# davidbau/rewriting

Measured on AMD Instinct MI355X. Metric: images/sec StyleGANv2-1024 fwd, higher is better.
Workload: dtype f32 (conv operands split into exact f16 pairs from 32x32 up, f32 accumulate); 1 GPU; stylegan2-1024 generator forward (FFHQ-1024 architecture); batch_per_gpu=64, mconv=seq, weights=synthetic seed 0, parallelism=seeds partitioned per rank, no collective, matrix_mode=split, direct_sums=auto

## Files before the change

include/rewriting_hip.h:

```cpp
#ifndef REWRITING_HIP_H
#define REWRITING_HIP_H

#include <stdint.h>

#ifdef __cplusplus
extern "C" {
#endif

typedef void* rw_stream_t;

#define RW_ERR_BAD_ARGUMENT 10001
#define RW_ERR_UNSUPPORTED  10002

int rw_abi_version(void);
const char* rw_error_string(int code);


int rw_fused_bias_act_f32(const float* x, const float* b, const float* ref, float* y,
                          int64_t n, int64_t step_b, int64_t size_b,
                          int act, int grad, float alpha, float scale, rw_stream_t stream);
int rw_fused_bias_act_f16(const uint16_t* x, const uint16_t* b, const uint16_t* ref, uint16_t* y,
                          int64_t n, int64_t step_b, int64_t size_b,
                          int act, int grad, float alpha, float scale, rw_stream_t stream);
int rw_fused_bias_act_f64(const double* x, const double* b, const double* ref, double* y,
// ... 9 lines not shown

int rw_upfirdn2d_f32(const float* x, const float* k, float* y,
                     int major, int in_h, int in_w, int minor, int kh, int kw,
                     int up_x, int up_y, int down_x, int down_y,
                     int pad_x0, int pad_x1, int pad_y0, int pad_y1, rw_stream_t stream);
int rw_upfirdn2d_f16(const uint16_t* x, const uint16_t* k, uint16_t* y,
                     int major, int in_h, int in_w, int minor, int kh, int kw,
                     int up_x, int up_y, int down_x, int down_y,
                     int pad_x0, int pad_x1, int pad_y0, int pad_y1, rw_stream_t stream);
int rw_upfirdn2d_f64(const double* x, const double* k, double* y,
                     int major, int in_h, int in_w, int minor, int kh, int kw,
                     int up_x, int up_y, int down_x, int down_y,
                     int pad_x0, int pad_x1, int pad_y0, int pad_y1, rw_stream_t stream);


int rw_pixel_norm_f32(const float* x, float* y, int batch, int dim, float eps, rw_stream_t stream);

int rw_equal_linear_f32(const float* x, const float* w, const float* bias, float* y,
                        int batch, int in_dim, int out_dim, int64_t x_stride,
                        float w_scale, float b_scale, int act, float alpha, float act_scale,
                        rw_stream_t stream);

int rw_adjust_latent_f32(const float* w, const float* avg, float* out, int batch, int n_latent,
                         int dim, float psi, rw_stream_t stream);

int rw_style_mul_f32(const float* x, const float* style, float* y, int batch, int channels,
                     int64_t hw, rw_stream_t stream);

int rw_weight_sqsum_f32(const float* w, float* wsq, int out_ch, int in_ch, int taps, float w_scale,
                        rw_stream_t stream);

int rw_demod_f32(const float* wsq, const float* style, float* demod, int batch, int out_ch,
                 int in_ch, float eps, rw_stream_t stream);

long long rw_packed_conv_weight_elems(int out_ch, int in_ch, int mode);
int rw_pack_conv_weight_f32(const float* w, float* wp, int out_ch, int in_ch, int mode,
                            rw_stream_t stream);

typedef struct rw_conv_epilogue {
  const float* style;
  const float* demod;
  const float* noise;
  const float* noise_w;
  const float* bias;
  int act;
} rw_conv_epilogue;

int rw_conv3x3_f32(const float* x, const float* wp, float* y, int batch, int in_ch, int out_ch,
                   int h, int w, float w_scale, const rw_conv_epilogue* ep, int impl,
                   rw_stream_t stream);

typedef struct rw_rgb_epilogue {
  const float* weight;
  const float* style;
  const float* bias;
  const float* skip;
  float* out;
  float scale;
} rw_rgb_epilogue;
int rw_conv3x3_to_rgb_f32(const float* x, const float* wp, float* y, int batch, int in_ch, int out_ch,
                          int h, int w, float w_scale, const rw_conv_epilogue* ep,
                          const rw_rgb_epilogue* rgb, rw_stream_t stream);

long long rw_packed_conv_weight_bf16x3_bytes(int out_ch, int in_ch);
int rw_pack_conv_weight_bf16x3(const float* w, void* wb, int out_ch, int in_ch, rw_stream_t stream);
int rw_conv3x3_bf16x6_f32(const float* x, const void* wb, float* y, int batch, int in_ch, int out_ch,
// ... 341 lines not shown
```

rewriting_amd/_lib.py:

```python
import ctypes
import os
from ctypes import (POINTER, Structure, c_char_p, c_double, c_float, c_int, c_int32, c_int64, c_uint,
                    c_void_p)

_HERE = os.path.dirname(os.path.abspath(__file__))
LIB_PATH = os.environ.get('RW_HIP_LIB') or os.path.join(_HERE, 'librewriting_hip.so')

ABI_VERSION = 11


class ConvEpilogue(Structure):
    _fields_ = [('style', c_void_p), ('demod', c_void_p), ('noise', c_void_p),
                ('noise_w', c_void_p), ('bias', c_void_p), ('act', c_int)]


class RgbEpilogue(Structure):
    _fields_ = [('weight', c_void_p), ('style', c_void_p), ('bias', c_void_p), ('skip', c_void_p),
                ('out', c_void_p), ('scale', c_float)]


LPIPS_MAX_TAPS = 8


class LpipsMaps(Structure):
    _fields_ = [('d', c_void_p * LPIPS_MAX_TAPS), ('h', c_int * LPIPS_MAX_TAPS), ('w', c_int * LPIPS_MAX_TAPS), ('n', c_int)]


LpipsGradMaps = LpipsMaps


class SolveProblem(Structure):
    _fields_ = [
        ('out_ch', c_int), ('in_ch', c_int), ('h', c_int), ('w', c_int), ('rank', c_int),
        ('key', c_void_p), ('style', c_void_p), ('val', c_void_p), ('bias', c_void_p),
        ('noise', c_void_p), ('noise_w', c_void_p), ('context', c_void_p), ('ortho', c_void_p),
        ('weight', c_void_p), ('exp_avg', c_void_p), ('exp_avg_sq', c_void_p),
        ('step_size', c_void_p), ('bc2_sqrt', c_void_p), ('step_counter', c_void_p),
        ('losses', c_void_p),
        ('conv', c_void_p), ('wsq', c_void_p), ('gd', c_void_p), ('c2', c_void_p),
        ('grad', c_void_p),
        ('ksplit', c_int), ('beta1', c_float), ('beta2', c_float), ('eps', c_float),
        ('w_scale', c_float), ('low_rank_gradient', c_int),
        ('one_minus_beta1', c_float), ('one_minus_beta2', c_float),
        ('upsample', c_int), ('blur_k', c_void_p), ('linear_insert', c_int), ('lambda_', c_void_p),
    ]


SIGNATURES = {
    'rw_abi_version': (c_int, []),
    'rw_error_string': (c_char_p, [c_int]),
    'rw_fused_bias_act_f32': (c_int, [c_void_p, c_void_p, c_void_p, c_void_p, c_int64, c_int64,
                                      c_int64, c_int, c_int, c_float, c_float, c_void_p]),
    'rw_fused_bias_act_f16': (c_int, [c_void_p, c_void_p, c_void_p, c_void_p, c_int64, c_int64,
                                      c_int64, c_int, c_int, c_float, c_float, c_void_p]),
    'rw_fused_bias_act_f64': (c_int, [c_void_p, c_void_p, c_void_p, c_void_p, c_int64, c_int64,
                                      c_int64, c_int, c_int, c_double, c_double, c_void_p]),
    'rw_bias_grad_f32': (c_int, [c_void_p, c_void_p, c_int64, c_int64, c_int64, c_void_p]),
    'rw_bias_grad_f16': (c_int, [c_void_p, c_void_p, c_int64, c_int64, c_int64, c_void_p]),
    'rw_bias_grad_f64': (c_int, [c_void_p, c_void_p, c_int64, c_int64, c_int64, c_void_p]),
    'rw_upfirdn2d_f32': (c_int, [c_void_p, c_void_p, c_void_p] + [c_int] * 14 + [c_void_p]),
    'rw_upfirdn2d_f16': (c_int, [c_void_p, c_void_p, c_void_p] + [c_int] * 14 + [c_void_p]),
    'rw_upfirdn2d_f64': (c_int, [c_void_p, c_void_p, c_void_p] + [c_int] * 14 + [c_void_p]),
    'rw_pixel_norm_f32': (c_int, [c_void_p, c_void_p, c_int, c_int, c_float, c_void_p]),
    'rw_equal_linear_f32': (c_int, [c_void_p, c_void_p, c_void_p, c_void_p, c_int, c_int, c_int,
                                    c_int64, c_float, c_float, c_int, c_float, c_float, c_void_p]),
    'rw_adjust_latent_f32': (c_int, [c_void_p, c_void_p, c_void_p, c_int, c_int, c_int, c_float,
                                     c_void_p]),
    'rw_style_mul_f32': (c_int, [c_void_p, c_void_p, c_void_p, c_int, c_int, c_int64, c_void_p]),
    'rw_weight_sqsum_f32': (c_int, [c_void_p, c_void_p, c_int, c_int, c_int, c_float, c_void_p]),
    'rw_demod_f32': (c_int, [c_void_p, c_void_p, c_void_p, c_int, c_int, c_int, c_float, c_void_p]),
    'rw_packed_conv_weight_elems': (ctypes.c_longlong, [c_int, c_int, c_int]),
    'rw_pack_conv_weight_f32': (c_int, [c_void_p, c_void_p, c_int, c_int, c_int, c_void_p]),
    'rw_conv3x3_f32': (c_int, [c_void_p, c_void_p, c_void_p, c_int, c_int, c_int, c_int, c_int,
                               c_float, POINTER(ConvEpilogue), c_int, c_void_p]),
    'rw_packed_conv_weight_bf16x3_bytes': (ctypes.c_longlong, [c_int, c_int]),
    'rw_pack_conv_weight_bf16x3': (c_int, [c_void_p, c_void_p, c_int, c_int, c_void_p]),
    'rw_conv3x3_bf16x6_f32': (c_int, [c_void_p, c_void_p, c_void_p, c_int, c_int, c_int, c_int, c_int,
                                      c_float, POINTER(ConvEpilogue), c_void_p]),
    'rw_conv3x3_to_rgb_f32': (c_int, [c_void_p, c_void_p, c_void_p, c_int, c_int, c_int, c_int, c_int,
                                      c_float, POINTER(ConvEpilogue), POINTER(RgbEpilogue), c_void_p]),
    'rw_conv_transpose3x3s2_f32': (c_int, [c_void_p, c_void_p, c_void_p, c_int, c_int, c_int, c_int,
                                           c_int, c_float, POINTER(ConvEpilogue), c_int, c_void_p]),
    'rw_noise_add_f32': (c_int, [c_void_p, c_void_p, c_void_p, c_void_p, c_int, c_int, c_int64,
                                 c_void_p]),
    'rw_blur_noise_act_f32': (c_int, [c_void_p, c_void_p, c_void_p, c_void_p, c_void_p, c_void_p,
                                      c_int, c_int, c_int, c_int, c_void_p]),
    'rw_to_rgb_f32': (c_int, [c_void_p, c_void_p, c_void_p, c_void_p, c_void_p, c_void_p, c_int,
                              c_int, c_int64, c_float, c_void_p]),
    'rw_second_moment_workspace_bytes': (c_int64, [c_int, c_int64]),
    'rw_second_moment_f32': (c_int, [c_void_p, c_void_p, c_int64, c_int, c_int64, c_int, c_void_p,
                                     c_void_p]),
    'rw_channel_sums_f32': (c_int, [c_void_p, c_void_p, c_int64, c_int, c_int64, c_int, c_int,
                                    c_void_p]),
    'rw_channel_moments_f32': (c_int, [c_void_p, c_void_p, c_int64, c_int, c_int64, c_int, c_int,
                                       c_void_p]),
    'rw_key_response_f32': (c_int, [c_void_p, c_void_p, c_void_p, c_void_p, c_int64, c_int, c_int64, c_int,
                                    c_void_p]),
    'rw_render_bytes_f32': (c_int, [c_void_p, c_void_p, c_void_p, c_int64, c_int, c_int, c_int, c_int, c_int, c_float,
                                    c_int, c_uint, c_int32, c_float, c_void_p]),
    'rw_png_segment_bytes': (c_int64, []),
    'rw_png_segment_capacity': (c_int64, []),
    'rw_png_table_words': (c_int64, []),
    'rw_png_filter_u8': (c_int, [c_void_p] * 6 + [c_int64, c_int, c_int, c_void_p]),
# ... 183 lines not shown
```

rewriting_amd/csrc/rw_ops.hip:

```cpp
#include "rw_common.h"
#include <stdlib.h>
#include <stdint.h>

extern "C" int rw_abi_version(void) { return 11; }

extern "C" const char* rw_error_string(int code) {
  if (code == 0) return "success";
  if (code == RW_ERR_BAD_ARGUMENT) return "rewriting_hip: bad argument";
  if (code == RW_ERR_UNSUPPORTED) return "rewriting_hip: unsupported configuration";
  return hipGetErrorString((hipError_t)code);
}

template <typename T> struct RwAcc { typedef T type; };
template <> struct RwAcc<_Float16> { typedef float type; };

template <typename A>
__device__ __forceinline__ A rw_bias_act_one(A x, A ref, int code, A alpha, A scale) {
  A y;
  switch (code) {
    default:
    case 10: y = x; break;
    case 11: y = x; break;
    case 12: y = A(0); break;
    case 30: y = (x > A(0)) ? x : x * alpha; break;
// ... 393 lines not shown
    wr[j] = (j < per && i < in_dim) ? w[(int64_t)o * in_dim + i] * w_scale : 0.f;
  }
  const float bv = bias ? bias[o] * b_scale : 0.f;
  for (int b0 = blockIdx.y * RW_LINEAR_ROWS; b0 < batch; b0 += gridDim.y * RW_LINEAR_ROWS) {
    float acc[RW_LINEAR_ROWS];
#pragma unroll
    for (int r = 0; r < RW_LINEAR_ROWS; ++r) {
      acc[r] = 0.f;
      const int b = b0 + r;
      if (b < batch) {
        const float* xr = x + (int64_t)b * x_stride;
#pragma unroll
        for (int j = 0; j < RW_LINEAR_MAX_PER_LANE; ++j) {
          const int i = lane + j * 64;
          if (j < per && i < in_dim) acc[r] += xr[i] * wr[j];
        }
      }
    }
#pragma unroll
    for (int off = 32; off > 0; off >>= 1)
#pragma unroll
      for (int r = 0; r < RW_LINEAR_ROWS; ++r) acc[r] += __shfl_xor(acc[r], off, 64);
    if (lane < RW_LINEAR_ROWS && b0 + lane < batch) {
      float v = acc[0];
#pragma unroll
      for (int r = 1; r < RW_LINEAR_ROWS; ++r) v = (lane == r) ? acc[r] : v;
      v += bv;
      if (act) v = ((v > 0.f) ? v : v * alpha) * act_scale;
      y[(int64_t)(b0 + lane) * out_dim + o] = v;
    }
  }
}

__global__ void __launch_bounds__(64) equal_linear_mfma_kernel(
    const float* __restrict__ x, const float* __restrict__ w, const float* __restrict__ bias,
    float* __restrict__ y, int batch, int in_dim, int out_dim, int64_t x_stride, float w_scale,
    float b_scale, int act, float alpha, float act_scale) {
  const int lane = threadIdx.x, mn = lane & 15, q = lane >> 4;
  const int o0 = blockIdx.x * 16, b0 = blockIdx.y * 16;
  const int brow = min(b0 + mn, batch - 1);
  const float* xp = x + (int64_t)brow * x_stride + 4 * q;
  const float* wp = w + (int64_t)(o0 + mn) * in_dim + 4 * q;
  rw_f32x4 acc = {0.f, 0.f, 0.f, 0.f};
  const int blocks = in_dim >> 4;
  constexpr int DEPTH = 8;
  for (int c0 = 0; c0 < blocks; c0 += DEPTH) {
    rw_f32x4 a[DEPTH], b[DEPTH];
#pragma unroll
    for (int d = 0; d < DEPTH; ++d) {
      const int c = min(c0 + d, blocks - 1);
      a[d] = *reinterpret_cast<const rw_f32x4*>(xp + 16 * c);
      b[d] = *reinterpret_cast<const rw_f32x4*>(wp + 16 * c);
    }
#pragma unroll
    for (int d = 0; d < DEPTH; ++d) {
      if (c0 + d < blocks) {
        const rw_f32x4 bs = b[d] * w_scale;
#pragma unroll
        for (int j = 0; j < 4; ++j) acc = __builtin_amdgcn_mfma_f32_16x16x4f32(a[d][j], bs[j], acc, 0, 0, 0);
      }
    }
  }
  const int o = o0 + mn;
  const float bv = bias ? bias[o] * b_scale : 0.f;
#pragma unroll
  for (int j = 0; j < 4; ++j) {
    const int b = b0 + 4 * q + j;
    if (b < batch) {
      float v = acc[j] + bv;
      if (act) v = ((v > 0.f) ? v : v * alpha) * act_scale;
      y[(int64_t)b * out_dim + o] = v;
    }
  }
}

extern "C" int rw_equal_linear_f32(const float* x, const float* w, const float* bias, float* y,
                                   int batch, int in_dim, int out_dim, int64_t x_stride,
                                   float w_scale, float b_scale, int act, float alpha,
                                   float act_scale, rw_stream_t stream) {
  RW_CHECK_ARG(x && w && y && batch > 0 && in_dim > 0 && out_dim > 0 && x_stride >= in_dim);
  const char* impl = getenv("RW_LINEAR_IMPL");
  const bool butterfly = impl && atoi(impl) == 1;
  if (!butterfly && in_dim % 16 == 0 && out_dim % 16 == 0 && x_stride % 4 == 0 && ((uintptr_t)x & 15) == 0 &&
      ((uintptr_t)w & 15) == 0) {
    hipLaunchKernelGGL(equal_linear_mfma_kernel, dim3(out_dim / 16, (batch + 15) / 16), dim3(64), 0, rw_s(stream), x,
                       w, bias, y, batch, in_dim, out_dim, x_stride, w_scale, b_scale, act, alpha, act_scale);
    return RW_LAUNCH_RESULT();
  }
  if (in_dim > 64 * RW_LINEAR_MAX_PER_LANE) return RW_ERR_UNSUPPORTED;
  int gy = (batch + RW_LINEAR_ROWS - 1) / RW_LINEAR_ROWS;
  if (gy > 64) gy = 64;
  hipLaunchKernelGGL(equal_linear_kernel, dim3((out_dim + 3) / 4, gy), dim3(256), 0, rw_s(stream), x, w,
                     bias, y, batch, in_dim, out_dim, x_stride, w_scale, b_scale, act, alpha,
                     act_scale);
  return RW_LAUNCH_RESULT();
}

__global__ void __launch_bounds__(256) adjust_latent_kernel(const float* __restrict__ w,
                                                            const float* __restrict__ avg,
                                                            float* __restrict__ out, int batch,
                                                            int n_latent, int dim, float psi) {
  const int64_t total = (int64_t)batch * n_latent * dim;
  for (int64_t idx = (int64_t)blockIdx.x * blockDim.x + threadIdx.x; idx < total;
       idx += (int64_t)gridDim.x * blockDim.x) {
    const int d = (int)(idx % dim);
    const int b = (int)(idx / ((int64_t)n_latent * dim));
    float v = w[(int64_t)b * dim + d];
    if (avg) { const float a = avg[d]; v = a + psi * (v - a); }
    out[idx] = v;
  }
}

extern "C" int rw_adjust_latent_f32(const float* w, const float* avg, float* out, int batch,
                                    int n_latent, int dim, float psi, rw_stream_t stream) {
  RW_CHECK_ARG(w && out && batch > 0 && n_latent > 0 && dim > 0);
  const int64_t total = (int64_t)batch * n_latent * dim;
  hipLaunchKernelGGL(adjust_latent_kernel, dim3(rw_stream_grid(total, 256)), dim3(256), 0,
// ... 61 lines not shown
       i += (int64_t)gridDim.x * blockDim.x) {
    float acc = 0.f;
    for (int t = 0; t < taps; ++t) { const float v = w_scale * w[i * taps + t]; acc += v * v; }
    wsq[i] = acc;
  }
}

extern "C" int rw_weight_sqsum_f32(const float* w, float* wsq, int out_ch, int in_ch, int taps,
                                   float w_scale, rw_stream_t stream) {
  RW_CHECK_ARG(w && wsq && out_ch > 0 && in_ch > 0 && taps > 0);
  const int64_t pairs = (int64_t)out_ch * in_ch;
  hipLaunchKernelGGL(weight_sqsum_kernel, dim3(rw_stream_grid(pairs, 256)), dim3(256), 0,
                     rw_s(stream), w, wsq, pairs, taps, w_scale);
  return RW_LAUNCH_RESULT();
}

__global__ void __launch_bounds__(256) demod_kernel(const float* __restrict__ wsq,
                                                    const float* __restrict__ style,
                                                    float* __restrict__ demod, int batch, int out_ch,
                                                    int in_ch, float eps) {
  const int64_t idx = (int64_t)blockIdx.x * 4 + (threadIdx.x >> 6);
  const int lane = threadIdx.x & 63;
  if (idx >= (int64_t)batch * out_ch) return;
  const int b = (int)(idx / out_ch), o = (int)(idx % out_ch);
  float acc = 0.f;
  for (int i = lane; i < in_ch; i += 64) {
    const float s = style[(int64_t)b * in_ch + i];
    acc += (s * s) * wsq[(int64_t)o * in_ch + i];
  }
  acc = rw_wave_sum(acc);
  if (lane == 0) demod[idx] = rsqrtf(acc + eps);
}

__global__ void __launch_bounds__(64) demod_mfma_kernel(const float* __restrict__ wsq, const float* __restrict__ style,
                                                        float* __restrict__ demod, int batch, int out_ch, int in_ch,
                                                        float eps) {
  const int lane = threadIdx.x, mn = lane & 15, q = lane >> 4;
  const int o0 = blockIdx.x * 16, b0 = blockIdx.y * 16;
  const int brow = min(b0 + mn, batch - 1);
  const float* sp = style + (int64_t)brow * in_ch + 4 * q;
  const float* wp = wsq + (int64_t)(o0 + mn) * in_ch + 4 * q;
  rw_f32x4 acc = {0.f, 0.f, 0.f, 0.f};
  const int blocks = in_ch >> 4;
  constexpr int DEPTH = 8;
  for (int c0 = 0; c0 < blocks; c0 += DEPTH) {
    rw_f32x4 a[DEPTH], b[DEPTH];
#pragma unroll
    for (int d = 0; d < DEPTH; ++d) {
      const int c = min(c0 + d, blocks - 1);
      a[d] = *reinterpret_cast<const rw_f32x4*>(sp + 16 * c);
      b[d] = *reinterpret_cast<const rw_f32x4*>(wp + 16 * c);
    }
#pragma unroll
    for (int d = 0; d < DEPTH; ++d) {
      if (c0 + d < blocks) {
#pragma unroll
        for (int j = 0; j < 4; ++j) acc = __builtin_amdgcn_mfma_f32_16x16x4f32(a[d][j] * a[d][j], b[d][j], acc, 0, 0, 0);
      }
    }
  }
#pragma unroll
  for (int j = 0; j < 4; ++j) {
    const int b = b0 + 4 * q + j;
    if (b < batch) demod[(int64_t)b * out_ch + o0 + mn] = rsqrtf(acc[j] + eps);
  }
}

extern "C" int rw_demod_f32(const float* wsq, const float* style, float* demod, int batch,
                            int out_ch, int in_ch, float eps, rw_stream_t stream) {
  RW_CHECK_ARG(wsq && style && demod && batch > 0 && out_ch > 0 && in_ch > 0);
  const char* impl = getenv("RW_LINEAR_IMPL");
  if (!(impl && atoi(impl) == 1) && in_ch % 16 == 0 && out_ch % 16 == 0 && ((uintptr_t)wsq & 15) == 0 &&
      ((uintptr_t)style & 15) == 0) {
    hipLaunchKernelGGL(demod_mfma_kernel, dim3(out_ch / 16, (batch + 15) / 16), dim3(64), 0, rw_s(stream), wsq, style,
                       demod, batch, out_ch, in_ch, eps);
    return RW_LAUNCH_RESULT();
  }
  const int64_t waves = (int64_t)batch * out_ch;
  hipLaunchKernelGGL(demod_kernel, dim3((unsigned)rw_cdiv(waves, 4)), dim3(256), 0, rw_s(stream),
                     wsq, style, demod, batch, out_ch, in_ch, eps);
  return RW_LAUNCH_RESULT();
}

__constant__ int rw_up_tap_order[9] = {0, 2, 6, 8, 1, 7, 3, 5, 4};

static inline bool rw_frag_ok(int out_ch, int in_ch) { return out_ch % 32 == 0 && in_ch % 16 == 0; }
static inline int rw_frag_ic(int out_ch, int mode) { return (mode == 1 || out_ch % 64 == 0) ? 16 : 8; }

extern "C" long long rw_packed_conv_weight_elems(int out_ch, int in_ch, int mode) {
  if (out_ch <= 0 || in_ch <= 0 || (mode != 0 && mode != 1)) return -1;
  const long long io = (long long)in_ch * out_ch;
  if (!rw_frag_ok(out_ch, in_ch)) return 9 * io;
  return 18 * io;
}

__global__ void __launch_bounds__(256) pack_conv_weight_kernel(const float* __restrict__ w,
                                                               float* __restrict__ wp, int out_ch,
                                                               int in_ch, int mode) {
  const int64_t total = (int64_t)9 * in_ch * out_ch;
  for (int64_t idx = (int64_t)blockIdx.x * blockDim.x + threadIdx.x; idx < total;
       idx += (int64_t)gridDim.x * blockDim.x) {
    const int o = (int)(idx % out_ch);
    const int i = (int)((idx / out_ch) % in_ch);
    const int slab = (int)(idx / ((int64_t)out_ch * in_ch));
    const int tap = mode == 0 ? slab : rw_up_tap_order[slab];
    wp[idx] = w[((int64_t)o * in_ch + i) * 9 + tap];
// ... 402 lines not shown
    for (int i = 0; i < in_ch; ++i) {
      const float v = xb[(int64_t)i * hw + q];
      a[0] += wm[i] * v; a[1] += wm[in_ch + i] * v; a[2] += wm[2 * in_ch + i] * v;
    }
#pragma unroll
    for (int c = 0; c < 3; ++c) {
      const int64_t off = ((int64_t)b * 3 + c) * hw + q;
      float o = a[c] + (bias ? bias[c] : 0.f);
      if (skip) o += skip[off];
      y[off] = o;
    }
  }
}

extern "C" int rw_to_rgb_f32(const float* x, const float* w, const float* style, const float* bias,
                             const float* skip, float* y, int batch, int in_ch, int64_t hw,
                             float w_scale, rw_stream_t stream) {
  RW_CHECK_ARG(x && w && style && y && batch > 0 && in_ch > 0 && hw > 0);
  if (hw % 4) {
    int gs = (int)rw_cdiv(hw, 256);
    if (gs > 2048) gs = 2048;
    hipLaunchKernelGGL(to_rgb_scalar_kernel, dim3(gs, batch), dim3(256), 3 * in_ch * sizeof(float), rw_s(stream), x, w,
                       style, bias, skip, y, in_ch, hw, w_scale);
    return RW_LAUNCH_RESULT();
  }
  int gx = (int)rw_cdiv(hw / 4, 256);
  const int cap = (256 * 8 + batch - 1) / batch;
  if (gx > cap) gx = cap;
  if (gx < 1) gx = 1;
  hipLaunchKernelGGL(to_rgb_kernel, dim3(gx, batch), dim3(256), 3 * in_ch * sizeof(float),
                     rw_s(stream), x, w, style, bias, skip, y, in_ch, hw, w_scale);
  return RW_LAUNCH_RESULT();
}
```

rewriting_amd/hip.py:

```python
import ctypes
from collections import namedtuple as _namedtuple

import torch

from . import _lib
from ._lib import ConvEpilogue, RgbEpilogue, SolveProblem, check

SQRT2 = 2 ** 0.5


def _stream():
    return ctypes.c_void_p(torch.cuda.current_stream().cuda_stream)


def _dev(t, name='tensor', dtype=torch.float32):
    if not isinstance(t, torch.Tensor):
        raise TypeError('%s must be a torch.Tensor' % name)
    if not t.is_cuda:
        raise RuntimeError('rewriting_amd: %s is on %s; the HIP kernels need a GPU tensor '
                           '(there is no CPU fallback)' % (name, t.device))
    if t.dtype != dtype:
        if dtype == torch.float32:
            raise RuntimeError('rewriting_amd: %s is %s; the C ABI is fp32 only (RW_ERR_UNSUPPORTED, include/rewriting_hip.h: '
                               'the reference\'s pybind modules also dispatch half and double, this library does not) -- '
# ... 200 lines not shown
    return y


def pixel_norm(x, eps=1e-8):
    return _pixel_norm_as(torch.float32, x, eps)


def equal_linear(x, weight, bias, w_scale, b_scale, act=False, alpha=0.2, act_scale=SQRT2):
    return _equal_linear_as(torch.float32, x, weight, bias, w_scale, b_scale, act, alpha, act_scale)


def adjust_latent(w, avg, n_latent, psi):
    return _adjust_latent_as(torch.float32, w, avg, n_latent, psi)


def style_mul(x, style):
    return _style_mul_as(torch.float32, x, style)


def weight_sqsum(weight, w_scale):
    return _weight_sqsum_as(torch.float32, weight, w_scale)


def demod(wsq, style, eps=1e-8):
    return _demod_as(torch.float32, wsq, style, eps)


def noise_add(x, noise, noise_w):
    return _noise_add_as(torch.float32, x, noise, noise_w)


def to_rgb(x, weight, style, bias, skip, w_scale):
    return _to_rgb_as(torch.float32, x, weight, style, bias, skip, w_scale)


def blur_noise_act(x, k4, noise, noise_w, bias, post_scale=None, y_amax=None):
    x = _dev(x, 'fmap')
    k4 = _dev(k4, 'blur kernel')
    noise = _opt(noise, 'noise')
    noise_w = _opt(noise_w, 'noise weight')
    bias = _opt(bias, 'bias')
    b, c, ih, iw = x.shape
    y = torch.empty(b, c, ih - 1, iw - 1, device=x.device, dtype=x.dtype)
    post_scale = _post_scale(post_scale, b, c, 'channels')
    y_amax = _amax_out(y_amax, y.numel())
    check(lib().rw_blur_noise_act_amax_f32(_p(x), _p(k4), _p(noise), _p(noise_w), _p(bias), _p(post_scale), _p(y),
                                           b, c, ih - 1, iw - 1, _p(y_amax), _stream()))
    return y


HalfSkip = _namedtuple('HalfSkip', 'image fir')


def _half_skip(skip, b, h, w):
    image, fir = _dev(skip.image, 'rgb skip (half size)'), _dev(skip.fir, 'upsampling kernel')
    if tuple(image.shape) != (b, 3, h // 2, w // 2) or h % 2 or w % 2 or tuple(fir.shape) != (4, 4):
        raise ValueError('half-size rgb skip / kernel shapes')
    return HalfSkip(image, fir)


def rgb_combine(partials, bias, skip):
    partials = _dev(partials, 'rgb partial sums')
    bias = _opt(bias, 'rgb bias')
    n, b, c, h, w = partials.shape
    y = torch.empty(b, 3, h, w, device=partials.device, dtype=partials.dtype)
    if isinstance(skip, HalfSkip):
# ... 1342 lines not shown
```

rewriting_amd/utils/stylegan2/models.py:

```python
import contextlib
import math
import re
import threading
import warnings
from collections import OrderedDict, namedtuple

import numpy as np
import torch
from torch import nn

from . import grad, op, routing
from .routing import switches
from ... import hip


_weight_epoch = [0]


def bump_weight_epoch():
    _weight_epoch[0] += 1


class _DerivedWeights:

# ... 1038 lines not shown
        k = list(self._modules).index('up_rgb%d' % (int(math.log2(from_res)) - 2))
        d = z
        for m in mods[:k]:
            d = m(d)
        total = d.latent.shape[0]
        out = None
        with _scope(final=final):
            for s in range(0, total, mb):
                e = min(s + mb, total)
                part = DataBag({key: (v[s:e] if torch.is_tensor(v) and v.dim() > 0 and v.shape[0] == total else v)
                                for key, v in d.items()})
                part['batch_rows'] = (s, total)
                for m in mods[k:]:
                    part = m(part)
                if out is None:
                    out = part.new_empty((total,) + tuple(part.shape[1:]))
                out[s:e] = part
                del part
        return out

    def _prefetch_modulations(self, d, aux):
        pre = {}
        todo = []
        for name, mod in self._modules.items():
            if not isinstance(mod, nn.Sequential) or isinstance(mod, StyledConvSeq):
                continue
            kids = list(mod.children())
            if len(kids) != 2 or not isinstance(kids[0], PickLatent):
                continue
            if isinstance(kids[1], StyledConvSeq) and kids[1]._fusable() and isinstance(kids[1].mconv, ModulatedConv2dSeq):
                todo.append((kids[0].index, kids[1]))
            elif isinstance(kids[1], ToRGBF):
                todo.append((kids[0].index, kids[1]))
        if len(todo) < 3:
            return {}
        main = torch.cuda.current_stream()
        aux.wait_stream(main)
        with torch.cuda.stream(aux):
            for index, mod in todo[2:]:
                lat = d.latent[:, index]
                if isinstance(mod, ToRGBF):
                    pre[id(mod)] = mod.conv.modulation(lat)
                else:
                    style = mod.mconv.modulation(DataBag(style=lat)).style
                    pre[id(mod)] = (style, mod.mconv.dconv.demod_factors(style))
        return dict(pre=pre, pre_join=aux)

    def _topology(self):
        near, final, prev = {}, None, None
        last = ('layer%d' % (self.num_layers + 1), 'to_rgb%d' % (self.log_size - 1))
        steps = list(self._modules.items())
        for (name, step), (nname, nstep) in zip(steps, steps[1:] + [(None, None)]):
            sconv = getattr(step, 'sconv', None)
            conv = sconv or getattr(step, 'conv', None)
            if not isinstance(conv, StyledConvSeq):
                continue
            if prev is not None:
                near[id(prev)] = near[id(prev)]._replace(reader=conv)
            prev = conv
            kids = list(nstep.children()) if nstep is not None else []
            picks = [m for m in kids if isinstance(m, PickLatent)]
            index = picks[0].index if len(picks) == 1 else None
            leads = index is not None and kids[0] is picks[0]
            nconv, rgb = getattr(nstep, 'sconv', None), getattr(nstep, 'rgb', None)
            successor = torgb = None
            if (conv is sconv and leads and isinstance(nconv, StyledConvSeq)
                    and getattr(conv.mconv, 'upsample', False) and not getattr(nconv.mconv, 'upsample', False)):
                successor = (nconv, index)
            if isinstance(rgb, ToRGBF):
                if leads and len(kids) == 2 and kids[1] is rgb:
                    torgb = (rgb, index)
                if conv is sconv and index is not None and (name, nname) == last:
                    final = (conv, rgb, index)
            near[id(conv)] = _Neighbours(None, successor, torgb)
        return near, final

    def bag_from_z(self, z):
        return InputLatent()(z)

# ... 48 lines not shown
```

rewriting_amd/utils/stylegan2/routing.py:

```python
import os
from collections import namedtuple

from ... import hip

_CONV_IMPLS = {'auto': 0, 'mfma': 0, 'direct': 1, 'generic': 2, 'halo': 3, 'nosplitk': 5}
ONE_PASS_UP_MAX_IN = 64
FUSED_UP_MAX_IN = 512

Switches = namedtuple('Switches', [
    'fuse',
    'conv_impl',
    'conv_precision',
    'conv_algo',
    'up_algo',
    'mm',
    'mm_hooked_split',
    'mm_parts',
    'mm_direct16',
    'micro_batch',
    'up_fused',
    'up_fused2',
    'up_fused2_hooked',
    'up_fused2_max_in',
    'up_fused2_join',
    'direct16_small',
    'direct16_hooked',
    'dconv_ws_fwd',
    'dconv_v',
    'rgb_partial',
    'rgb_f4',
    'rgb_stream',
    'strip_stream',
    'side_priority',
    'prescale',
    'mm_no_handover',
    'prefetch_styles',
    'fuse_final_rgb',
    'rgb_inline_up',
])


def switches():
    env = os.environ.get
    direct16 = env('RW_MM_DIRECT16', 'auto')
    parts = env('RW_MM_PARTS')
    k, _, res = env('RW_MICRO_BATCH', '0').partition(':')
    return Switches(
        fuse=env('RW_FUSE', '1') != '0',
        conv_impl=_CONV_IMPLS[env('RW_CONV_IMPL', 'auto')],
        conv_precision=env('RW_CONV_PRECISION', 'f32'),
        conv_algo=env('RW_CONV_ALGO'),
        up_algo=env('RW_UP_ALGO', 'winograd'),
        mm=env('RW_MM'),
        mm_hooked_split=env('RW_MM_HOOKED', 'split') != 'f32',
        mm_parts=None if parts is None else tuple(parts.split(',')),
        mm_direct16={'auto': ('conv', 'up'), '1': ('conv', 'up', 'rgb')}.get(direct16) or tuple(direct16.split(',')),
        micro_batch=(int(k or 0), int(res or 256)),
        up_fused=env('RW_UP_FUSED', '1') != '0',
        up_fused2=env('RW_UP_FUSED2', '1') == '1',
        up_fused2_hooked=env('RW_UP_FUSED2_HOOKED', '1') == '1',
        up_fused2_max_in=int(env('RW_UP_FUSED2_MAX_IN', FUSED_UP_MAX_IN)),
        up_fused2_join=env('RW_UP_FUSED2_JOIN') == '1',
        direct16_small=env('RW_DIRECT16_SMALL', '1') != '0',
        direct16_hooked=env('RW_DIRECT16_HOOKED', '1') == '1',
        dconv_ws_fwd=env('RW_DCONV_WS_FWD', '1') != '0',
        dconv_v=env('RW_DCONV_V') == '1',
        rgb_partial=env('RW_RGB_PARTIAL', '1') != '0',
        rgb_f4=env('RW_RGB_F4', '1') != '0',
        rgb_stream=env('RW_RGB_STREAM', '1') != '0',
        strip_stream=env('RW_STRIP_STREAM', '1') != '0',
        side_priority=int(env('RW_SIDE_PRIORITY', '0')),
        prescale=env('RW_PRESCALE', '1') != '0',
        mm_no_handover=env('RW_MM_NO_HANDOVER') == '1',
        prefetch_styles=env('RW_PREFETCH_STYLES', '1') != '0',
        fuse_final_rgb=env('RW_FUSE_FINAL_RGB', '1') != '0',
        rgb_inline_up=env('RW_RGB_INLINE_UP', '1') != '0',
    )


Context = namedtuple('Context', 'image_path on_device capturing rgb_stream aux_stream weight_changes')

STRIDE1_KERNELS = ('direct16', 'wino4_split', 'wino4', 'wino', 'bf16x6', 'gemm')
WHOLE_LAYER_KERNELS = ('fused', 'one_pass_direct16', 'one_pass_wino4')
UP_KERNELS = WHOLE_LAYER_KERNELS + ('f22_strips', 'halo_strips', 'plain')

Stride1Route = namedtuple('Stride1Route', 'kernel specialised rgb_partials reads_bound reports_bound prescaled')

UpRoute = namedtuple('UpRoute', 'kernel split side_strips reads_bound runs_layer')

FinalRgbRoute = namedtuple('FinalRgbRoute', 'kernel reads_bound')


def _stride1(kernel, *flags):
    if kernel not in STRIDE1_KERNELS:
        raise ValueError(kernel)
    return Stride1Route(kernel, *flags)


def _up(kernel, *flags):
    if kernel not in UP_KERNELS:
        raise ValueError(kernel)
    return UpRoute(kernel, *flags, kernel in WHOLE_LAYER_KERNELS)


def _final_rgb(kernel, reads_bound):
    if kernel not in STRIDE1_KERNELS:
        raise ValueError(kernel)
# ... 96 lines not shown
```

Measured before the change: 1656 images/sec.

## Batch all style modulation linears and demod factors into grouped kernel launches

Adds grouped kernels that compute every layer's style linear, and every demodulation factor, in a single launch each. A prefix table of tiles tells each block which problem it belongs to. The prefetch path is switched on by default, and it replaces the earlier side-stream prefetch of per-layer modulations. The goal is to cut the many small kernel launches and the Python overhead in the modulation stage. In exchange, the parameter struct passed to the kernel is large, and the per-block problem lookup adds a little work.

```diff
diff --git a/include/rewriting_hip.h b/include/rewriting_hip.h
--- a/include/rewriting_hip.h
+++ b/include/rewriting_hip.h
@@ -65,6 +65,39 @@
 
 int rw_demod_f32(const float* wsq, const float* style, float* demod, int batch, int out_ch,
                  int in_ch, float eps, rw_stream_t stream);
+
+#define RW_GROUP_MAX 32
+typedef struct RwLinearGroup {
+  const float* x[RW_GROUP_MAX];
+  const float* w[RW_GROUP_MAX];
+  const float* bias[RW_GROUP_MAX];
+  float* y[RW_GROUP_MAX];
+  int64_t x_stride[RW_GROUP_MAX];
+  int in_dim[RW_GROUP_MAX];
+  int out_dim[RW_GROUP_MAX];
+  float w_scale[RW_GROUP_MAX];
+  float b_scale[RW_GROUP_MAX];
+  int act[RW_GROUP_MAX];
+  int tile0[RW_GROUP_MAX + 1];
+  int n;
+  int batch;
+  float alpha;
+  float act_scale;
+} RwLinearGroup;
+int rw_equal_linear_group_f32(const RwLinearGroup* g, rw_stream_t stream);
+
+typedef struct RwDemodGroup {
+  const float* wsq[RW_GROUP_MAX];
+  const float* style[RW_GROUP_MAX];
+  float* demod[RW_GROUP_MAX];
+  int out_ch[RW_GROUP_MAX];
+  int in_ch[RW_GROUP_MAX];
+  int tile0[RW_GROUP_MAX + 1];
+  int n;
+  int batch;
+  float eps;
+} RwDemodGroup;
+int rw_demod_group_f32(const RwDemodGroup* g, rw_stream_t stream);
 
 long long rw_packed_conv_weight_elems(int out_ch, int in_ch, int mode);
 int rw_pack_conv_weight_f32(const float* w, float* wp, int out_ch, int in_ch, int mode,
diff --git a/rewriting_amd/_lib.py b/rewriting_amd/_lib.py
--- a/rewriting_amd/_lib.py
+++ b/rewriting_amd/_lib.py
@@ -17,6 +17,24 @@
 class RgbEpilogue(Structure):
     _fields_ = [('weight', c_void_p), ('style', c_void_p), ('bias', c_void_p), ('skip', c_void_p),
                 ('out', c_void_p), ('scale', c_float)]
+
+
+ERR_UNSUPPORTED = 10002
+GROUP_MAX = 32
+
+
+class LinearGroup(Structure):
+    _fields_ = [('x', c_void_p * GROUP_MAX), ('w', c_void_p * GROUP_MAX), ('bias', c_void_p * GROUP_MAX),
+                ('y', c_void_p * GROUP_MAX), ('x_stride', c_int64 * GROUP_MAX), ('in_dim', c_int * GROUP_MAX),
+                ('out_dim', c_int * GROUP_MAX), ('w_scale', c_float * GROUP_MAX), ('b_scale', c_float * GROUP_MAX),
+                ('act', c_int * GROUP_MAX), ('tile0', c_int * (GROUP_MAX + 1)), ('n', c_int), ('batch', c_int),
+                ('alpha', c_float), ('act_scale', c_float)]
+
+
+class DemodGroup(Structure):
+    _fields_ = [('wsq', c_void_p * GROUP_MAX), ('style', c_void_p * GROUP_MAX), ('demod', c_void_p * GROUP_MAX),
+                ('out_ch', c_int * GROUP_MAX), ('in_ch', c_int * GROUP_MAX), ('tile0', c_int * (GROUP_MAX + 1)),
+                ('n', c_int), ('batch', c_int), ('eps', c_float)]
 
 
 LPIPS_MAX_TAPS = 8
@@ -69,6 +87,8 @@
     'rw_style_mul_f32': (c_int, [c_void_p, c_void_p, c_void_p, c_int, c_int, c_int64, c_void_p]),
     'rw_weight_sqsum_f32': (c_int, [c_void_p, c_void_p, c_int, c_int, c_int, c_float, c_void_p]),
     'rw_demod_f32': (c_int, [c_void_p, c_void_p, c_void_p, c_int, c_int, c_int, c_float, c_void_p]),
+    'rw_equal_linear_group_f32': (c_int, [POINTER(LinearGroup), c_void_p]),
+    'rw_demod_group_f32': (c_int, [POINTER(DemodGroup), c_void_p]),
     'rw_packed_conv_weight_elems': (ctypes.c_longlong, [c_int, c_int, c_int]),
     'rw_pack_conv_weight_f32': (c_int, [c_void_p, c_void_p, c_int, c_int, c_int, c_void_p]),
     'rw_conv3x3_f32': (c_int, [c_void_p, c_void_p, c_void_p, c_int, c_int, c_int, c_int, c_int,
diff --git a/rewriting_amd/csrc/rw_ops.hip b/rewriting_amd/csrc/rw_ops.hip
--- a/rewriting_amd/csrc/rw_ops.hip
+++ b/rewriting_amd/csrc/rw_ops.hip
@@ -449,12 +449,10 @@
   }
 }
 
-__global__ void __launch_bounds__(64) equal_linear_mfma_kernel(
-    const float* __restrict__ x, const float* __restrict__ w, const float* __restrict__ bias,
-    float* __restrict__ y, int batch, int in_dim, int out_dim, int64_t x_stride, float w_scale,
-    float b_scale, int act, float alpha, float act_scale) {
+__device__ __forceinline__ void equal_linear_mfma_tile(const float* x, const float* w, const float* bias, float* y,
+                                                       int batch, int in_dim, int out_dim, int64_t x_stride, float w_scale,
+                                                       float b_scale, int act, float alpha, float act_scale, int o0, int b0) {
   const int lane = threadIdx.x, mn = lane & 15, q = lane >> 4;
-  const int o0 = blockIdx.x * 16, b0 = blockIdx.y * 16;
   const int brow = min(b0 + mn, batch - 1);
   const float* xp = x + (int64_t)brow * x_stride + 4 * q;
   const float* wp = w + (int64_t)(o0 + mn) * in_dim + 4 * q;
@@ -491,15 +489,30 @@
   }
 }
 
+__global__ void __launch_bounds__(64) equal_linear_mfma_kernel(
+    const float* __restrict__ x, const float* __restrict__ w, const float* __restrict__ bias,
+    float* __restrict__ y, int batch, int in_dim, int out_dim, int64_t x_stride, float w_scale,
+    float b_scale, int act, float alpha, float act_scale) {
+  equal_linear_mfma_tile(x, w, bias, y, batch, in_dim, out_dim, x_stride, w_scale, b_scale, act, alpha, act_scale,
+                         blockIdx.x * 16, blockIdx.y * 16);
+}
+
+static inline bool rw_linear_mfma_ok(const float* x, const float* w, int in_dim, int out_dim, int64_t x_stride) {
+  return in_dim % 16 == 0 && out_dim % 16 == 0 && x_stride % 4 == 0 && ((uintptr_t)x & 15) == 0 &&
+         ((uintptr_t)w & 15) == 0;
+}
+
+static inline bool rw_linear_butterfly_forced() {
+  const char* impl = getenv("RW_LINEAR_IMPL");
+  return impl && atoi(impl) == 1;
+}
+
 extern "C" int rw_equal_linear_f32(const float* x, const float* w, const float* bias, float* y,
                                    int batch, int in_dim, int out_dim, int64_t x_stride,
                                    float w_scale, float b_scale, int act, float alpha,
                                    float act_scale, rw_stream_t stream) {
   RW_CHECK_ARG(x && w && y && batch > 0 && in_dim > 0 && out_dim > 0 && x_stride >= in_dim);
-  const char* impl = getenv("RW_LINEAR_IMPL");
-  const bool butterfly = impl && atoi(impl) == 1;
-  if (!butterfly && in_dim % 16 == 0 && out_dim % 16 == 0 && x_stride % 4 == 0 && ((uintptr_t)x & 15) == 0 &&
-      ((uintptr_t)w & 15) == 0) {
+  if (!rw_linear_butterfly_forced() && rw_linear_mfma_ok(x, w, in_dim, out_dim, x_stride)) {
     hipLaunchKernelGGL(equal_linear_mfma_kernel, dim3(out_dim / 16, (batch + 15) / 16), dim3(64), 0, rw_s(stream), x,
                        w, bias, y, batch, in_dim, out_dim, x_stride, w_scale, b_scale, act, alpha, act_scale);
     return RW_LAUNCH_RESULT();
@@ -627,11 +640,9 @@
   if (lane == 0) demod[idx] = rsqrtf(acc + eps);
 }
 
-__global__ void __launch_bounds__(64) demod_mfma_kernel(const float* __restrict__ wsq, const float* __restrict__ style,
-                                                        float* __restrict__ demod, int batch, int out_ch, int in_ch,
-                                                        float eps) {
+__device__ __forceinline__ void demod_mfma_tile(const float* wsq, const float* style, float* demod, int batch, int out_ch,
+                                                int in_ch, float eps, int o0, int b0) {
   const int lane = threadIdx.x, mn = lane & 15, q = lane >> 4;
-  const int o0 = blockIdx.x * 16, b0 = blockIdx.y * 16;
   const int brow = min(b0 + mn, batch - 1);
   const float* sp = style + (int64_t)brow * in_ch + 4 * q;
   const float* wp = wsq + (int64_t)(o0 + mn) * in_ch + 4 * q;
@@ -661,12 +672,20 @@
   }
 }
 
+__global__ void __launch_bounds__(64) demod_mfma_kernel(const float* __restrict__ wsq, const float* __restrict__ style,
+                                                        float* __restrict__ demod, int batch, int out_ch, int in_ch,
+                                                        float eps) {
+  demod_mfma_tile(wsq, style, demod, batch, out_ch, in_ch, eps, blockIdx.x * 16, blockIdx.y * 16);
+}
+
+static inline bool rw_demod_mfma_ok(const float* wsq, const float* style, int out_ch, int in_ch) {
+  return in_ch % 16 == 0 && out_ch % 16 == 0 && ((uintptr_t)wsq & 15) == 0 && ((uintptr_t)style & 15) == 0;
+}
+
 extern "C" int rw_demod_f32(const float* wsq, const float* style, float* demod, int batch,
                             int out_ch, int in_ch, float eps, rw_stream_t stream) {
   RW_CHECK_ARG(wsq && style && demod && batch > 0 && out_ch > 0 && in_ch > 0);
-  const char* impl = getenv("RW_LINEAR_IMPL");
-  if (!(impl && atoi(impl) == 1) && in_ch % 16 == 0 && out_ch % 16 == 0 && ((uintptr_t)wsq & 15) == 0 &&
-      ((uintptr_t)style & 15) == 0) {
+  if (!rw_linear_butterfly_forced() && rw_demod_mfma_ok(wsq, style, out_ch, in_ch)) {
     hipLaunchKernelGGL(demod_mfma_kernel, dim3(out_ch / 16, (batch + 15) / 16), dim3(64), 0, rw_s(stream), wsq, style,
                        demod, batch, out_ch, in_ch, eps);
     return RW_LAUNCH_RESULT();
@@ -1135,3 +1154,60 @@
                      rw_s(stream), x, w, style, bias, skip, y, in_ch, hw, w_scale);
   return RW_LAUNCH_RESULT();
 }
+
+
+__device__ __forceinline__ int rw_group_problem(const int* tile0, int n, int t) {
+  int p = 0;
+  while (p + 1 < n && t >= tile0[p + 1]) ++p;
+  return p;
+}
+
+__device__ __forceinline__ int rw_group_out(const RwLinearGroup& g, int p) { return g.out_dim[p]; }
+__device__ __forceinline__ int rw_group_out(const RwDemodGroup& g, int p) { return g.out_ch[p]; }
+
+__device__ __forceinline__ void rw_group_tile(const RwLinearGroup& g, int p, int o0, int b0) {
+  equal_linear_mfma_tile(g.x[p], g.w[p], g.bias[p], g.y[p], g.batch, g.in_dim[p], g.out_dim[p], g.x_stride[p],
+                         g.w_scale[p], g.b_scale[p], g.act[p], g.alpha, g.act_scale, o0, b0);
+}
+
+__device__ __forceinline__ void rw_group_tile(const RwDemodGroup& g, int p, int o0, int b0) {
+  demod_mfma_tile(g.wsq[p], g.style[p], g.demod[p], g.batch, g.out_ch[p], g.in_ch[p], g.eps, o0, b0);
+}
+
+template <typename Group>
+__global__ void __launch_bounds__(64) mod_group_kernel(const Group g) {
+  const int p = rw_group_problem(g.tile0, g.n, blockIdx.x);
+  const int t = blockIdx.x - g.tile0[p];
+  const int out_tiles = rw_group_out(g, p) >> 4;
+  rw_group_tile(g, p, (t % out_tiles) * 16, (t / out_tiles) * 16);
+}
+
+static inline bool rw_group_tiles_ok(const int* tile0, int i, int batch, int out_dim) {
+  return tile0[i + 1] - tile0[i] == (out_dim / 16) * ((batch + 15) / 16);
+}
+
+extern "C" int rw_equal_linear_group_f32(const RwLinearGroup* g, rw_stream_t stream) {
+  RW_CHECK_ARG(g && g->n > 0 && g->batch > 0);
+  if (g->n > RW_GROUP_MAX || rw_linear_butterfly_forced()) return RW_ERR_UNSUPPORTED;
+  RW_CHECK_ARG(g->tile0[0] == 0);
+  for (int i = 0; i < g->n; ++i) {
+    RW_CHECK_ARG(g->x[i] && g->w[i] && g->y[i] && g->in_dim[i] > 0 && g->out_dim[i] > 0 && g->x_stride[i] >= g->in_dim[i]);
+    if (!rw_linear_mfma_ok(g->x[i], g->w[i], g->in_dim[i], g->out_dim[i], g->x_stride[i])) return RW_ERR_UNSUPPORTED;
+    RW_CHECK_ARG(rw_group_tiles_ok(g->tile0, i, g->batch, g->out_dim[i]));
+  }
+  hipLaunchKernelGGL(mod_group_kernel<RwLinearGroup>, dim3(g->tile0[g->n]), dim3(64), 0, rw_s(stream), *g);
+  return RW_LAUNCH_RESULT();
+}
+
+extern "C" int rw_demod_group_f32(const RwDemodGroup* g, rw_stream_t stream) {
+  RW_CHECK_ARG(g && g->n > 0 && g->batch > 0);
+  if (g->n > RW_GROUP_MAX || rw_linear_butterfly_forced()) return RW_ERR_UNSUPPORTED;
+  RW_CHECK_ARG(g->tile0[0] == 0);
+  for (int i = 0; i < g->n; ++i) {
+    RW_CHECK_ARG(g->wsq[i] && g->style[i] && g->demod[i] && g->out_ch[i] > 0 && g->in_ch[i] > 0);
+    if (!rw_demod_mfma_ok(g->wsq[i], g->style[i], g->out_ch[i], g->in_ch[i])) return RW_ERR_UNSUPPORTED;
+    RW_CHECK_ARG(rw_group_tiles_ok(g->tile0, i, g->batch, g->out_ch[i]));
+  }
+  hipLaunchKernelGGL(mod_group_kernel<RwDemodGroup>, dim3(g->tile0[g->n]), dim3(64), 0, rw_s(stream), *g);
+  return RW_LAUNCH_RESULT();
+}
diff --git a/rewriting_amd/hip.py b/rewriting_amd/hip.py
--- a/rewriting_amd/hip.py
+++ b/rewriting_amd/hip.py
@@ -256,6 +256,116 @@
 
 def to_rgb(x, weight, style, bias, skip, w_scale):
     return _to_rgb_as(torch.float32, x, weight, style, bias, skip, w_scale)
+
+
+GROUP_MAX = _lib.GROUP_MAX
+
+StyleEntry = _namedtuple('StyleEntry', 'index weight bias w_scale b_scale act', defaults=(False,))
+
+
+def group_tile_prefix(batch, out_dims):
+    tile0 = [0]
+    for out_dim in out_dims:
+        tile0.append(tile0[-1] + (out_dim // 16) * ((batch + 15) // 16))
+    return tile0
+
+
+def group_chunks(n):
+    return [range(s, min(s + GROUP_MAX, n)) for s in range(0, n, GROUP_MAX)]
+
+
+def _group_struct(cls, batch, fields, problems, out_field, **shared):
+    g = cls(n=len(problems), batch=batch, **shared)
+    for k, problem in enumerate(problems):
+        for name, value in zip(fields, problem):
+            getattr(g, name)[k] = value
+    tile0 = group_tile_prefix(batch, [p[fields.index(out_field)] for p in problems])
+    g.tile0[:len(tile0)] = tile0
+    return g
+
+
+_LINEAR_FIELDS = ('x', 'w', 'bias', 'y', 'x_stride', 'in_dim', 'out_dim', 'w_scale', 'b_scale', 'act')
+_DEMOD_FIELDS = ('wsq', 'style', 'demod', 'out_ch', 'in_ch')
+
+
+def linear_group_struct(batch, problems, alpha=0.2, act_scale=SQRT2):
+    return _group_struct(_lib.LinearGroup, batch, _LINEAR_FIELDS, problems, 'out_dim', alpha=alpha, act_scale=act_scale)
+
+
+def demod_group_struct(batch, problems, eps=1e-8):
+    return _group_struct(_lib.DemodGroup, batch, _DEMOD_FIELDS, problems, 'out_ch', eps=eps)
+
+
+def _f32_on_device(*tensors):
+    return all(isinstance(t, torch.Tensor) and t.is_cuda and t.dtype == torch.float32 for t in tensors if t is not None)
+
+
+def _grouped(shapes, device, launch, one_by_one):
+    sizes = [b * o for b, o in shapes]
+    flat = torch.empty(sum(sizes), device=device, dtype=torch.float32)
+    outs, start = [], 0
+    for size, shape in zip(sizes, shapes):
+        outs.append(flat[start:start + size].view(shape))
+        start += size
+    for ids in group_chunks(len(shapes)):
+        code = launch(ids, outs)
+        if code == _lib.ERR_UNSUPPORTED:
+            for i, out in zip(ids, one_by_one(ids)):
+                outs[i] = out
+        else:
+            check(code)
+    return outs
+
+
+def style_group(latent, entries):
+    entries = [StyleEntry(*e) for e in entries]
+    rows = [latent if e.index is None else latent[:, e.index] for e in entries]
+
+    def one_by_one(ids):
+        return [equal_linear(rows[i], entries[i].weight, entries[i].bias, entries[i].w_scale, entries[i].b_scale,
+                             act=entries[i].act) for i in ids]
+    if not entries:
+        return []
+    if not (_f32_on_device(latent, *(t for e in entries for t in (e.weight, e.bias)))
+            and all(r.ndim == 2 and r.stride(1) == 1 and e.weight.ndim == 2 and e.weight.shape[1] == r.shape[1]
+                    and (e.bias is None or e.bias.numel() == e.weight.shape[0]) for r, e in zip(rows, entries))):
+        return one_by_one(range(len(entries)))
+    rows = [r.detach() for r in rows]
+    weights = [_dev(e.weight, 'weight') for e in entries]
+    biases = [_opt(e.bias, 'bias') for e in entries]
+    batch = latent.shape[0]
+
+    def launch(ids, outs):
+        problems = []
+        for i in ids:
+            out_dim, in_dim = weights[i].shape
+            x_stride = rows[i].stride(0) if batch > 1 else in_dim
+            problems.append((rows[i].data_ptr(), weights[i].data_ptr(), None if biases[i] is None else biases[i].data_ptr(),
+                             outs[i].data_ptr(), max(x_stride, in_dim), in_dim, out_dim, float(entries[i].w_scale),
+                             float(entries[i].b_scale), int(bool(entries[i].act))))
+        return lib().rw_equal_linear_group_f32(ctypes.byref(linear_group_struct(batch, problems)), _stream())
+    return _grouped([(batch, w.shape[0]) for w in weights], latent.device, launch, one_by_one)
+
+
+def demod_group(entries, eps=1e-8):
+    entries = list(entries)
+
+    def one_by_one(ids):
+        return [demod(entries[i][0], entries[i][1], eps) for i in ids]
+    if not entries:
+        return []
+    batch = entries[0][1].shape[0]
+    if not (_f32_on_device(*(t for e in entries for t in e))
+            and all(w.ndim == 2 and tuple(s.shape) == (batch, w.shape[1]) for w, s in entries)):
+        return one_by_one(range(len(entries)))
+    wsqs = [_dev(w, 'wsq') for w, _ in entries]
+    styles = [_dev(s, 'style') for _, s in entries]
+
+    def launch(ids, outs):
+        problems = [(wsqs[i].data_ptr(), styles[i].data_ptr(), outs[i].data_ptr(), wsqs[i].shape[0], wsqs[i].shape[1])
+                    for i in ids]
+        return lib().rw_demod_group_f32(ctypes.byref(demod_group_struct(batch, problems, eps)), _stream())
+    return _grouped([(batch, w.shape[0]) for w in wsqs], styles[0].device, launch, one_by_one)
 
 
 def blur_noise_act(x, k4, noise, noise_w, bias, post_scale=None, y_amax=None):
diff --git a/rewriting_amd/utils/stylegan2/models.py b/rewriting_amd/utils/stylegan2/models.py
--- a/rewriting_amd/utils/stylegan2/models.py
+++ b/rewriting_amd/utils/stylegan2/models.py
@@ -1094,6 +1094,8 @@
                 todo.append((kids[0].index, kids[1]))
             elif isinstance(kids[1], ToRGBF):
                 todo.append((kids[0].index, kids[1]))
+        if _switches().mod_group:
+            return self._grouped_modulations(d.latent, todo)
         if len(todo) < 3:
             return {}
         main = torch.cuda.current_stream()
@@ -1107,6 +1109,18 @@
                     style = mod.mconv.modulation(DataBag(style=lat)).style
                     pre[id(mod)] = (style, mod.mconv.dconv.demod_factors(style))
         return dict(pre=pre, pre_join=aux)
+
+    @staticmethod
+    def _grouped_modulations(latent, todo):
+        linears = [mod.conv.modulation if isinstance(mod, ToRGBF) else mod.mconv.modulation for _, mod in todo]
+        styles = hip.style_group(latent, [(index, lin.weight, lin.bias, lin.scale, lin.lr_mul, bool(lin.activation))
+                                          for (index, _), lin in zip(todo, linears)])
+        demodulated = [(mod, style) for (_, mod), style in zip(todo, styles)
+                       if isinstance(mod, StyledConvSeq) and mod.mconv.dconv.demodulate]
+        factors = hip.demod_group([(mod.mconv.dconv.squared_sums(), style) for mod, style in demodulated])
+        demod = {id(mod): factor for (mod, _), factor in zip(demodulated, factors)}
+        return dict(pre={id(mod): style if isinstance(mod, ToRGBF) else (style, demod.get(id(mod)))
+                         for (_, mod), style in zip(todo, styles)})
 
     def _topology(self):
         near, final, prev = {}, None, None
diff --git a/rewriting_amd/utils/stylegan2/routing.py b/rewriting_amd/utils/stylegan2/routing.py
--- a/rewriting_amd/utils/stylegan2/routing.py
+++ b/rewriting_amd/utils/stylegan2/routing.py
@@ -35,6 +35,7 @@
     'prescale',
     'mm_no_handover',
     'prefetch_styles',
+    'mod_group',
     'fuse_final_rgb',
     'rgb_inline_up',
 ])
@@ -73,6 +74,7 @@
         prescale=env('RW_PRESCALE', '1') != '0',
         mm_no_handover=env('RW_MM_NO_HANDOVER') == '1',
         prefetch_styles=env('RW_PREFETCH_STYLES', '1') != '0',
+        mod_group=env('RW_MOD_GROUP', '1') != '0',
         fuse_final_rgb=env('RW_FUSE_FINAL_RGB', '1') != '0',
         rgb_inline_up=env('RW_RGB_INLINE_UP', '1') != '0',
     )
```

Result: no change. 1672 images/sec, median of 6 (+1.0%).
